# chrischoy/DeepGlobalRegistration

Hardware: AMD Instinct MI355X
Metric: pair registrations/sec (FCGF x2 + 1-NN + 6-D inlier net + gate + weighted Procrustes + SE(3) refinement) (higher is better)
Workload: dtype f32 results via 2 x f16 split operands (3 f16 MFMA products per MAC, f32 accumulate); k = 1 convs, kNN re-evaluation and registration in exact f32, SVD in f64

## Files before the change

### deepglobalregistration_amd/csrc/coordmap.hip

```cpp
#include <algorithm>

#include "dgr_internal.h"
#include "hash.h"

constexpr int SCAN_THREADS = 256;
constexpr int SCAN_ITEMS = 8;
constexpr int SCAN_BLOCK = SCAN_THREADS * SCAN_ITEMS;

__device__ __forceinline__ int block_exclusive_scan_256(int v, int *lds , int *total) {
  const int lane = threadIdx.x & 63, wave = threadIdx.x >> 6;
  int x = v;
#pragma unroll
  for (int d = 1; d < 64; d <<= 1) {
    int y = __shfl_up(x, d, 64);
    if (lane >= d) x += y;
  }
  if (lane == 63) lds[wave] = x;
  __syncthreads();
  int base = 0, tot = 0;
#pragma unroll
  for (int w = 0; w < SCAN_THREADS / 64; ++w) {
    int s = lds[w];
    if (w < wave) base += s;
    tot += s;
// ... 239 lines not shown
                            mask_out, stream);
  if (nc == 7)
    return unique_rows_t<7>(arena, keys, nullptr, n, first_flag, rank, n_unique_dev, table_out,
                            mask_out, stream);
  dgr_set_error("unsupported coordinate width %d", nc);
  return DGR_EINVAL;
}

template <int NC>
static int build_coord_maps_t(DgrArena &arena, const int32_t *coords, int64_t N, DgrMapSet *ms,
                              hipStream_t stream) {
  DgrCoordMap &c1 = ms->cm[0];
  c1.coords = const_cast<int32_t *>(coords);
  c1.n_cap = N;
  c1.ts = 1;
  DGR_ALLOC(c1.n_dev, arena, int32_t, 1);
  int32_t n32 = (int32_t)N;
  DGR_HIP_CHECK(hipMemcpyAsync(c1.n_dev, &n32, sizeof(int32_t), hipMemcpyHostToDevice, stream));
  {
    uint32_t cap = dgr_next_pow2((uint64_t)(2 * N > 64 ? 2 * N : 64));
    DGR_ALLOC(c1.table, arena, int32_t, cap);
    c1.table_mask = cap - 1;
    DGR_HIP_CHECK(hipMemsetAsync(c1.table, 0xff, (size_t)cap * sizeof(int32_t), stream));
    unique_insert<NC><<<grid_for(N), 256, 0, stream>>>(coords, nullptr, N, c1.table, cap - 1);
    unique_flag<NC><<<grid_for(N), 256, 0, stream>>>(coords, nullptr, N, c1.table, cap - 1, nullptr,
                                                    ms->overflow);
    DGR_LAUNCH_CHECK();
  }
  for (int l = 1; l < 4; ++l) {
    DgrCoordMap &p = ms->cm[l - 1];
    DgrCoordMap &c = ms->cm[l];
    c.ts = p.ts * 2;
    c.n_cap = p.n_cap;
    int32_t *keys, *flag, *rank;
    DGR_ALLOC(keys, arena, int32_t, p.n_cap * NC);
    DGR_ALLOC(flag, arena, int32_t, p.n_cap);
    DGR_ALLOC(rank, arena, int32_t, p.n_cap);
    DGR_ALLOC(c.coords, arena, int32_t, c.n_cap * NC);
    DGR_ALLOC(c.n_dev, arena, int32_t, 1);
    stride_keys<NC><<<grid_for(p.n_cap), 256, 0, stream>>>(p.coords, p.n_dev, c.ts, keys);
    DGR_CHECK(unique_rows_t<NC>(arena, keys, p.n_dev, p.n_cap, flag, rank, c.n_dev, &c.table,
                                &c.table_mask, stream));
    unique_compact<NC><<<grid_for(p.n_cap), 256, 0, stream>>>(keys, p.n_dev, p.n_cap, flag, rank,
                                                             c.coords, nullptr);
    table_relabel<<<grid_for((int64_t)c.table_mask + 1), 256, 0, stream>>>(c.table, c.table_mask + 1,
                                                                           rank);
    DGR_LAUNCH_CHECK();
  }
  return DGR_OK;
}

__global__ void half_keys_kernel(const int32_t *__restrict__ coords7, const int32_t *n_dev,
                                 int32_t *__restrict__ keys4) {
  int64_t r = (int64_t)blockIdx.x * blockDim.x + threadIdx.x;
  if (r >= *n_dev) return;
#pragma unroll
  for (int d = 0; d < 4; ++d) keys4[r * 4 + d] = coords7[r * 7 + d];
}

__global__ void bucket_count_kernel(const int32_t *__restrict__ keys4, const int32_t *n_dev,
                                    const int32_t *__restrict__ table, uint32_t mask,
                                    const int32_t *__restrict__ bkeys, int32_t *__restrict__ row_bucket,
                                    int32_t *counts) {
  int64_t r = (int64_t)blockIdx.x * blockDim.x + threadIdx.x;
  if (r >= *n_dev) return;
  int32_t q[4] = {keys4[r * 4], keys4[r * 4 + 1], keys4[r * 4 + 2], keys4[r * 4 + 3]};
  const int b = dgr_lookup<4>(table, mask, bkeys, q);
  row_bucket[r] = b;
  atomicAdd(&counts[b], 1);
}

__global__ void bucket_members_kernel(const int32_t *__restrict__ row_bucket, const int32_t *n_dev,
                                      const int32_t *__restrict__ start, int32_t *cursor, int32_t *__restrict__ members) {
  int64_t r = (int64_t)blockIdx.x * blockDim.x + threadIdx.x;
  if (r >= *n_dev) return;
  const int b = row_bucket[r];
  members[start[b] + atomicAdd(&cursor[b], 1)] = (int32_t)r;
}

__global__ void bucket_fill_kernel(const int32_t *__restrict__ row_bucket, const int32_t *n_dev,
                                   const int32_t *__restrict__ start, int32_t *cursor,
                                   const int32_t *__restrict__ members,
                                   const int32_t *__restrict__ coords7, int4 *__restrict__ second,
                                   int32_t *__restrict__ coords_new, int32_t *__restrict__ canon, int32_t *__restrict__ inv) {
  int64_t r = (int64_t)blockIdx.x * blockDim.x + threadIdx.x;
  if (r >= *n_dev) return;
  const int b = row_bucket[r];
  const int32_t *c = coords7 + r * 7;
  int p;
  if (members) {
    int rank = 0;
    for (int e = start[b], end = start[b + 1]; e < end; ++e) rank += members[e] < (int32_t)r;
    p = start[b] + rank;
  } else {
    p = start[b] + atomicAdd(&cursor[b], 1);
  }
  if (coords_new) {
#pragma unroll
    for (int d = 0; d < 7; ++d) coords_new[(int64_t)p * 7 + d] = c[d];
    canon[p] = (int32_t)r;
    inv[r] = p;
    second[p] = make_int4(c[4], c[5], c[6], p);
  } else {
    second[p] = make_int4(c[4], c[5], c[6], (int32_t)r);
  }
}

struct RenumberJobs {
  const int32_t *inv[4];
  int32_t *table[4];
  uint32_t cap[4];
};
__global__ void renumber_table_kernel(RenumberJobs j) {
  const int l = blockIdx.y;
  const uint32_t s = blockIdx.x * blockDim.x + threadIdx.x;
  if (s >= j.cap[l]) return;
  const int v = j.table[l][s];
  if (v >= 0) j.table[l][s] = j.inv[l][v];
}

int dgr_build_half_buckets(DgrArena &arena, DgrCoordMap *cm, DgrHalfBuckets *hb, int levels, int renumber_from,
                           hipStream_t stream) {
  DGR_REQUIRE(levels >= 1 && levels <= 4 && renumber_from >= 1, "half buckets: %d levels", levels);
  int32_t *keys[4], *flag[4], *rank[4], *nb_dev[4], *row_bucket[4], *counts[4], *cursor[4];
  uint32_t cap[4];
  size_t table_words = 0, count_words = 0;
  for (int l = 0; l < levels; ++l) {
    const int64_t n = cm[l].n_cap;
    cap[l] = dgr_next_pow2((uint64_t)(2 * n > 64 ? 2 * n : 64));
    table_words += cap[l];
    count_words += 2 * (size_t)(n + 1);
  }
  int32_t *tables, *cnts;
  DGR_ALLOC(tables, arena, int32_t, table_words);
  DGR_ALLOC(cnts, arena, int32_t, count_words);
  DGR_HIP_CHECK(hipMemsetAsync(tables, 0xff, table_words * sizeof(int32_t), stream));
  DGR_HIP_CHECK(hipMemsetAsync(cnts, 0, count_words * sizeof(int32_t), stream));
  for (int l = 0; l < levels; ++l) {
    const int64_t n = cm[l].n_cap;
    hb[l].table = tables; tables += cap[l];
    hb[l].mask = cap[l] - 1;
    counts[l] = cnts; cursor[l] = cnts + (n + 1); cnts += 2 * (n + 1);
    DGR_ALLOC(keys[l], arena, int32_t, n * 4);
    DGR_ALLOC(flag[l], arena, int32_t, n);
    DGR_ALLOC(rank[l], arena, int32_t, n);
    DGR_ALLOC(nb_dev[l], arena, int32_t, 1);
    DGR_ALLOC(row_bucket[l], arena, int32_t, n);
    DGR_ALLOC(hb[l].bkeys, arena, int32_t, n * 4);
    DGR_ALLOC(hb[l].start, arena, int32_t, n + 1);
    DGR_ALLOC(hb[l].second, arena, int4, n);
  }
  for (int l = 0; l < levels; ++l) {
    const int64_t n = cm[l].n_cap;
    half_keys_kernel<<<grid_for(n), 256, 0, stream>>>(cm[l].coords, cm[l].n_dev, keys[l]);
    unique_insert<4><<<grid_for(n), 256, 0, stream>>>(keys[l], cm[l].n_dev, n, hb[l].table, hb[l].mask);
    unique_flag<4><<<grid_for(n), 256, 0, stream>>>(keys[l], cm[l].n_dev, n, hb[l].table, hb[l].mask, flag[l], nullptr);
  }
  DGR_LAUNCH_CHECK();
  {
    const int32_t *ins[4];
    int32_t *outs[4], *tots[4];
    int64_t ns[4];
    for (int l = 0; l < levels; ++l) { ins[l] = flag[l]; outs[l] = rank[l]; tots[l] = nb_dev[l]; ns[l] = cm[l].n_cap; }
    DGR_CHECK(dgr_exclusive_scan_multi(arena, levels, ins, outs, ns, tots, stream));
  }
  for (int l = 0; l < levels; ++l) {
    const int64_t n = cm[l].n_cap;
    unique_compact<4><<<grid_for(n), 256, 0, stream>>>(keys[l], cm[l].n_dev, n, flag[l], rank[l], hb[l].bkeys, nullptr);
    table_relabel<<<grid_for((int64_t)hb[l].mask + 1), 256, 0, stream>>>(hb[l].table, hb[l].mask + 1, rank[l]);
    bucket_count_kernel<<<grid_for(n), 256, 0, stream>>>(keys[l], cm[l].n_dev, hb[l].table, hb[l].mask, hb[l].bkeys, row_bucket[l],
                                                         counts[l]);
  }
  DGR_LAUNCH_CHECK();
  {
    const int32_t *ins[4];
    int32_t *outs[4], *tots[4];
    int64_t ns[4];
    for (int l = 0; l < levels; ++l) { ins[l] = counts[l]; outs[l] = hb[l].start; tots[l] = nullptr; ns[l] = cm[l].n_cap + 1; }
    DGR_CHECK(dgr_exclusive_scan_multi(arena, levels, ins, outs, ns, tots, stream));
  }
  RenumberJobs rj = {};
  int nrj = 0;
  int64_t max_cap = 0;
  for (int l = 0; l < levels; ++l) {
    const int64_t n = cm[l].n_cap;
    int32_t *coords_new = nullptr, *canon = nullptr, *inv = nullptr;
    if (l >= renumber_from) {
      DGR_ALLOC(coords_new, arena, int32_t, n * 7);
      DGR_ALLOC(canon, arena, int32_t, n);
      DGR_ALLOC(inv, arena, int32_t, n);
      rj.inv[nrj] = inv; rj.table[nrj] = cm[l].table; rj.cap[nrj] = cm[l].table_mask + 1;
      max_cap = std::max<int64_t>(max_cap, rj.cap[nrj]);
      ++nrj;
    }
    const int32_t *members = nullptr;
    if (coords_new) {
      bucket_members_kernel<<<grid_for(n), 256, 0, stream>>>(row_bucket[l], cm[l].n_dev, hb[l].start, cursor[l], rank[l]);
      members = rank[l];
    }
    bucket_fill_kernel<<<grid_for(n), 256, 0, stream>>>(row_bucket[l], cm[l].n_dev, hb[l].start, cursor[l], members,
                                                        cm[l].coords, hb[l].second, coords_new, canon, inv);
    if (coords_new) { cm[l].coords = coords_new; cm[l].canon = canon; }
    hb[l].built = true;
  }
  if (nrj) renumber_table_kernel<<<dim3((unsigned)grid_for(max_cap), nrj), 256, 0, stream>>>(rj);
  DGR_LAUNCH_CHECK();
  return DGR_OK;
}

int dgr_build_coord_maps(DgrArena &arena, const int32_t *coords, int64_t N, DgrMapSet *ms,
                         hipStream_t stream) {
  if (ms->nc == 4) return build_coord_maps_t<4>(arena, coords, N, ms, stream);
  if (ms->nc == 7) return build_coord_maps_t<7>(arena, coords, N, ms, stream);
  dgr_set_error("unsupported dimension D=%d (3 and 6 are on the DGR path)", ms->D);
  return DGR_EINVAL;
}

template <typename T>
__global__ void voxel_keys(const T *__restrict__ xyz, int64_t M, T inv_unused, T voxel, int32_t batch,
                           int32_t *__restrict__ keys) {
  int64_t r = (int64_t)blockIdx.x * blockDim.x + threadIdx.x;
  if (r >= M) return;
  keys[r * 4] = batch;
#pragma unroll
  for (int d = 0; d < 3; ++d) keys[r * 4 + 1 + d] = (int32_t)floor(xyz[r * 3 + d] / voxel);
}

template <typename T>
__global__ void voxel_gather_xyz(const T *__restrict__ xyz, const int64_t *__restrict__ sel,
                                 const int32_t *n_dev, float *__restrict__ out) {
  int64_t r = (int64_t)blockIdx.x * blockDim.x + threadIdx.x;
  if (r >= *n_dev) return;
  int64_t s = sel[r];
#pragma unroll
  for (int d = 0; d < 3; ++d) out[r * 3 + d] = (float)xyz[s * 3 + d];
}

extern "C" int dgr_voxelize(dgr_ctx *ctx, const void *xyz, int is_f64, int64_t M, double voxel_size,
                            int32_t batch_index, int64_t *sel_out, int32_t *coords_out,
                            float *xyz_out, int64_t *n_out, dgr_stream stream_) {
  DGR_REQUIRE(ctx && xyz && sel_out && coords_out && n_out, "dgr_voxelize: NULL argument");
  DGR_REQUIRE(M > 0 && M < (1ll << 30), "dgr_voxelize: M=%lld out of range", (long long)M);
  DGR_REQUIRE(voxel_size > 0, "dgr_voxelize: voxel_size must be positive");
  hipStream_t stream = (hipStream_t)stream_;
  DGR_HIP_CHECK(hipSetDevice(ctx->device));
  DGR_CHECK(ctx->arena.reset());
  DgrArena &A = ctx->arena;
  int32_t *keys, *flag, *rank, *n_dev, *table;
  uint32_t mask;
  DGR_ALLOC(keys, A, int32_t, M * 4);
  DGR_ALLOC(flag, A, int32_t, M);
  DGR_ALLOC(rank, A, int32_t, M);
  DGR_ALLOC(n_dev, A, int32_t, 1);
  if (is_f64)
    voxel_keys<double><<<grid_for(M), 256, 0, stream>>>((const double *)xyz, M, 0.0, voxel_size,
                                                       batch_index, keys);
  else
    voxel_keys<float><<<grid_for(M), 256, 0, stream>>>((const float *)xyz, M, 0.f, (float)voxel_size,
                                                      batch_index, keys);
  DGR_CHECK(unique_rows_t<4>(A, keys, nullptr, M, flag, rank, n_dev, &table, &mask, stream));
  unique_compact<4><<<grid_for(M), 256, 0, stream>>>(keys, nullptr, M, flag, rank, coords_out, sel_out);
  if (xyz_out) {
    if (is_f64)
      voxel_gather_xyz<double><<<grid_for(M), 256, 0, stream>>>((const double *)xyz, sel_out, n_dev,
                                                               xyz_out);
    else
      voxel_gather_xyz<float><<<grid_for(M), 256, 0, stream>>>((const float *)xyz, sel_out, n_dev,
                                                              xyz_out);
  }
  DGR_LAUNCH_CHECK();
  int32_t n32 = 0;
  DGR_HIP_CHECK(hipMemcpyAsync(&n32, n_dev, sizeof(int32_t), hipMemcpyDeviceToHost, stream));
  DGR_HIP_CHECK(hipStreamSynchronize(stream));
  *n_out = n32;
  return DGR_OK;
}
```

### deepglobalregistration_amd/csrc/dgr_internal.h

```cpp
#pragma once
#include <hip/hip_runtime.h>
#include <stdint.h>
#include <stdio.h>
#include <stdlib.h>
#include <string>
#include <vector>

#include "../../include/dgr_hip.h"

void dgr_set_error(const char *fmt, ...);

#define DGR_HIP_CHECK(expr)                                                                  \
  do {                                                                                       \
    hipError_t _e = (expr);                                                                  \
    if (_e != hipSuccess) {                                                                  \
      dgr_set_error("%s:%d: %s failed: %s", __FILE__, __LINE__, #expr, hipGetErrorString(_e)); \
      return DGR_EHIP;                                                                       \
    }                                                                                        \
  } while (0)

#define DGR_CHECK(expr)          \
  do {                           \
    int _r = (expr);             \
    if (_r != DGR_OK) return _r; \
  } while (0)

#define DGR_REQUIRE(cond, ...)     \
  do {                             \
    if (!(cond)) {                 \
      dgr_set_error(__VA_ARGS__);  \
      return DGR_EINVAL;           \
    }                              \
  } while (0)

#define DGR_LAUNCH_CHECK() DGR_HIP_CHECK(hipGetLastError())

inline bool dgr_exact_f32() {
  static const bool on = getenv("DGR_EXACT_F32") != nullptr;
  return on;
}

struct DgrArena {
  struct Chunk {
    char *base;
    size_t size;
  };
  std::vector<Chunk> chunks;
  size_t cur = 0;
  size_t offset = 0;
  size_t high_water = 0, used_total = 0;
  uint64_t generation = 0;

  struct Mark {
    size_t cur, offset, used_total;
  };
  Mark mark() const { return {cur, offset, used_total}; }
  void rewind(const Mark &m) { cur = m.cur; offset = m.offset; used_total = m.used_total; }
  void *alloc(size_t bytes);
  int reset();
  void release();
  size_t reserved() const;
  template <typename T>
  T *get(size_t n) {
    return static_cast<T *>(alloc(n * sizeof(T)));
  }
};

#define DGR_ALLOC(ptr, arena, T, n)                       \
  do {                                                    \
    (ptr) = (arena).get<T>((size_t)(n) > 0 ? (size_t)(n) : 1); \
    if (!(ptr)) return DGR_ENOMEM;                        \
  } while (0)

constexpr int DGR_TILE_M = 64;

struct DgrCoordMap {
  int32_t *coords = nullptr;
  int32_t *n_dev = nullptr;
  int64_t n_cap = 0;
  int ts = 1;
  int32_t *table = nullptr;
  uint32_t table_mask = 0;
  int32_t *canon = nullptr;
};

struct DgrHalfBuckets {
  int32_t *bkeys = nullptr;
  int32_t *table = nullptr;
  uint32_t mask = 0;
  int32_t *start = nullptr;
  int4 *second = nullptr;
  bool built = false;
};

struct DgrKernelMap {
  int K = 0;
  int32_t *rule_ptr = nullptr;
  int32_t *tile_ptr = nullptr;
  int4 *tile_desc = nullptr;
  int64_t tile_cap = 0;
  int32_t *pair_in = nullptr;
  int32_t *pair_out = nullptr;
  int32_t *out_ptr = nullptr, *out_pos = nullptr;
  uint16_t *pair_k = nullptr;
  int32_t *in_ptr = nullptr, *in_pos = nullptr;
  int64_t pair_cap = 0;
  bool built = false;
};

constexpr int DGR_OS_ROWS = 64;
struct DgrNbrTable {
  int32_t *nbr = nullptr;
  int64_t n_pad = 0;
  int K = 27;
  bool built = false;
  int32_t *perm = nullptr, *cls_count = nullptr;
  int64_t cls_cap = 0;
};

struct DgrMapSet {
  int D = 3, nc = 4, conv1_ks = 3;
  bool use_nbr = false;
  DgrNbrTable nsame[4];
  DgrNbrTable ndown[3];
  DgrNbrTable nup[3];
  DgrCoordMap cm[4];
  DgrHalfBuckets hb[4];
  DgrKernelMap same[4];
  DgrKernelMap conv1;
  DgrKernelMap down[3];
  int32_t *overflow = nullptr;
};

int dgr_build_maps(DgrArena &arena, const int32_t *coords, int64_t N, int D, int conv1_ks,
                   DgrMapSet *ms, hipStream_t stream, bool skip_conv1_map = false, bool lean = false,
                   bool nbr_tables = false);
int dgr_nbr_counts(const DgrNbrTable &t, const int32_t *n_out_dev, int64_t counts[27]);
int dgr_conv1_probe(DgrArena &arena, const DgrCoordMap &cm, int ks, const float *in, int in_ld, int cin,
                    const float *w_tiled, const float *shift, float *out, int out_ld, int32_t *pair_count,
                    hipStream_t stream, const float *w_compact = nullptr, const char **kernel_name = nullptr,
                    uint32_t *out_amax = nullptr);
int dgr_unique_rows(DgrArena &arena, const int32_t *keys, int64_t n, int nc, int32_t *first_flag,
                    int32_t *rank, int32_t *n_unique_dev, int32_t **table_out, uint32_t *mask_out,
                    hipStream_t stream);
int dgr_exclusive_scan_i32(DgrArena &arena, const int32_t *in, int32_t *out, int64_t n,
                           int32_t *total_out, hipStream_t stream);
constexpr int DGR_SCAN_MAX = 24;
int dgr_exclusive_scan_multi(DgrArena &arena, int count, const int32_t *const *in, int32_t *const *out, const int64_t *n,
                             int32_t *const *total_out, hipStream_t stream);

struct DgrConvLaunch {
  const float *in;
  int in_ld;
  int in_relu;
  float *out;
  int out_ld;
  float *y;
  const float *shift;
  const float *w;
  int cin, cin_pad, cout, cout_pad, K;
  const int32_t *pair_in, *pair_out, *tile_ptr, *rule_ptr;
  const int4 *tile_desc;
  const int32_t *n_rows_dev;
  int64_t tile_bound;
  int l2_normalize = 0;
  unsigned long long *clk = nullptr;
};
int dgr_conv_launch(const DgrConvLaunch &a, int num_cus, hipStream_t stream, const char **kernel_name = nullptr);
struct DgrSplitRows {
  unsigned char *planes = nullptr;
  float *scale = nullptr;
  int channels = 0;
};
bool dgr_conv_wide_supported(int cin_pad, int cin, int cout);
// ... 136 lines not shown
```

### deepglobalregistration_amd/csrc/kmap.hip

```cpp
#include <string.h>

#include <algorithm>

#include "dgr_internal.h"
#include "hash.h"

constexpr int KM_THREADS = 256;

template <int D>
__device__ __forceinline__ void offset_of(int k, int ks, int ts, int32_t *delta) {
  const int half = ks >> 1;
#pragma unroll
  for (int d = 0; d < D; ++d) {
    delta[d] = ((k % ks) - half) * ts;
    k /= ks;
  }
}

template <int D>
__device__ __forceinline__ int probe(const int32_t *__restrict__ out_coords, int64_t o,
                                     const int32_t *delta, const int32_t *__restrict__ in_coords,
                                     const int32_t *__restrict__ in_table, uint32_t in_mask) {
  constexpr int NC = D + 1;
  int32_t q[NC];
// ... 19 lines not shown
  int32_t delta[D];
  offset_of<D>(k, ks, ts_in, delta);
  const int64_t o = (int64_t)rb * KM_THREADS + threadIdx.x;
  int hit = -1;
  if (o < n_out) {
    hit = probe<D>(out_coords, o, delta, in_coords, in_table, in_mask);
    hits[(int64_t)k * n_cap + o] = hit;
    if (hit >= 0) {
      atomicOr(&mask_out[o * KW + (k >> 5)], 1u << (k & 31));
      if (mask_in) atomicOr(&mask_in[(int64_t)hit * KW + (k >> 5)], 1u << (k & 31));
    }
  }
  unsigned long long m = __ballot(hit >= 0);
  if ((threadIdx.x & 63) == 0) wave_cnt[threadIdx.x >> 6] = __popcll(m);
  __syncthreads();
  if (threadIdx.x == 0) {
    int s = 0;
#pragma unroll
    for (int w = 0; w < KM_THREADS / 64; ++w) s += wave_cnt[w];
    block_counts[(int64_t)k * RB + rb] = s;
  }
}

__device__ __forceinline__ int mask_rank(const uint32_t *__restrict__ m, int k) {
  int r = 0;
  const int w = k >> 5;
  for (int i = 0; i < w; ++i) r += __popc(m[i]);
  return r + __popc(m[w] & ((1u << (k & 31)) - 1u));
}

__global__ void mask_count_kernel(const uint32_t *__restrict__ mask, int KW, const int32_t *n_dev, int64_t n_cap,
                                  int32_t *__restrict__ cnt, unsigned short *__restrict__ wpre = nullptr) {
  const int64_t r = (int64_t)blockIdx.x * blockDim.x + threadIdx.x;
  if (r >= n_cap) return;
  int c = 0;
  if (r < *n_dev)
    for (int i = 0; i < KW; ++i) {
      if (wpre) wpre[r * KW + i] = (unsigned short)c;
      c += __popc(mask[r * KW + i]);
    }
  cnt[r] = c;
}
constexpr int KM_MC_JOBS = 8;
struct MaskCountJobs {
  const uint32_t *mask[KM_MC_JOBS];
  const int32_t *n_dev[KM_MC_JOBS];
  long long n_cap[KM_MC_JOBS];
  int32_t *cnt[KM_MC_JOBS];
  unsigned short *wpre[KM_MC_JOBS];
};
template <int KW>
__global__ void mask_count_multi(MaskCountJobs J) {
  const int m = blockIdx.y;
  const int64_t r = (int64_t)blockIdx.x * blockDim.x + threadIdx.x;
  if (r >= J.n_cap[m]) return;
  int c = 0;
  if (r < *J.n_dev[m]) {
    uint32_t w[KW];
#pragma unroll
    for (int i = 0; i < KW; ++i) w[i] = J.mask[m][r * KW + i];
#pragma unroll
    for (int i = 0; i < KW; ++i) {
      J.wpre[m][r * KW + i] = (unsigned short)c;
      c += __popc(w[i]);
    }
  }
  J.cnt[m][r] = c;
}
__device__ __forceinline__ int mask_rank_pre(const uint32_t *__restrict__ m, const unsigned short *__restrict__ pre, int k) {
  return pre[k >> 5] + __popc(m[k >> 5] & ((1u << (k & 31)) - 1u));
}


__device__ __forceinline__ unsigned long long hit_pack(int k, int64_t o, int64_t in) {
  return ((unsigned long long)k << 54) | ((unsigned long long)o << 27) | (unsigned long long)in;
}
constexpr int KM_REGION = 512;
constexpr int KM_JOBS6 = 8;
struct HitList {
  unsigned long long *recs;
  int32_t *wave_count;
  int region;
};
__device__ __forceinline__ void hit_begin(volatile int *cur) {
  if ((threadIdx.x & 63) == 0) cur[threadIdx.x >> 6] = 0;
}
__device__ __forceinline__ int64_t hit_slots(int n, const HitList &h, volatile int *cur, int wave_id) {
  const unsigned long long act = __ballot(1), two = __ballot(n == 2);
  const int lane = threadIdx.x & 63, w = threadIdx.x >> 6;
  const unsigned long long below = (1ull << lane) - 1ull;
  int base = 0;
  if (lane == __ffsll((long long)act) - 1) {
    base = cur[w];
    const int need = __popcll(act) + __popcll(two);
    if (base >= 0 && base + need <= h.region) {
      cur[w] = base + need;
    } else {
      cur[w] = -1;
      base = -1;
    }
  }
  base = __builtin_amdgcn_readfirstlane(base);
  if (base < 0) return -1;
  return (int64_t)wave_id * h.region + base + __popcll(act & below) + __popcll(two & below);
}
__device__ __forceinline__ void hit_end(const HitList &h, volatile int *cur, int wave_id) {
  if ((threadIdx.x & 63) == 0) h.wave_count[wave_id] = cur[threadIdx.x >> 6];
}

struct PrunedArgs {
  const int32_t *out_coords, *n_out_dev;
  const int4 *out_order;
  int64_t n_cap;
  DgrHalfBuckets hb;
  int ts_in, symmetric;
};
template <class Emit>
__device__ __forceinline__ void pruned_search6(const PrunedArgs &a, int64_t t, Emit &&emit) {
  const int NJ = a.symmetric ? 14 : 27;
  const int ts_in = a.ts_in;
  const int ja = (int)(t / a.n_cap);
  const int64_t p = t - (int64_t)ja * a.n_cap;
  int b = -1;
  int64_t o = 0;
  int c4 = 0, c5 = 0, c6 = 0;
  if (ja < NJ && p < *a.n_out_dev) {
    const int4 me = a.out_order[p];
    o = me.w; c4 = me.x; c5 = me.y; c6 = me.z;
    const int32_t *co = a.out_coords + o * 7;
    int32_t q[4];
    q[0] = co[0];
    q[1] = co[1] + ((ja % 3) - 1) * ts_in;
    q[2] = co[2] + (((ja / 3) % 3) - 1) * ts_in;
    q[3] = co[3] + ((ja / 9) - 1) * ts_in;
    b = dgr_lookup<4>(a.hb.table, a.hb.mask, a.hb.bkeys, q);
  }
  const int beg = b >= 0 ? a.hb.start[b] : 0, end = b >= 0 ? a.hb.start[b + 1] : 0;
  for (int p0 = beg; p0 < end; p0 += 4) {
    int4 e[4];
#pragma unroll
    for (int u = 0; u < 4; ++u) e[u] = a.hb.second[min(p0 + u, end - 1)];
#pragma unroll
    for (int u = 0; u < 4; ++u) {
      if (p0 + u >= end) break;
      const int d4 = e[u].x - c4, d5 = e[u].y - c5, d6 = e[u].z - c6;
      if (abs(d4) <= ts_in && abs(d5) <= ts_in && abs(d6) <= ts_in) {
        const int k = ja + 27 * ((d4 / ts_in + 1) + 3 * (d5 / ts_in + 1) + 9 * (d6 / ts_in + 1));
        if (a.symmetric && ja == 13 && k > 364) continue;
        emit(k, o, e[u].w);
      }
    }
  }
}

struct Bits6Jobs {
  PrunedArgs pa[KM_JOBS6];
  uint32_t *mask_out[KM_JOBS6], *mask_in[KM_JOBS6];
  HitList hl[KM_JOBS6];
  int blocks[KM_JOBS6];
};
__global__ void __launch_bounds__(KM_THREADS)
    kmap_bits_pruned6(Bits6Jobs J, int KW) {
  __shared__ int hit_cur[KM_THREADS / 64];
  const int jm = blockIdx.y;
  if ((int)blockIdx.x >= J.blocks[jm]) return;
  const PrunedArgs a = J.pa[jm];
  uint32_t *const mask_out = J.mask_out[jm], *const mask_in = J.mask_in[jm];
  const HitList hl = J.hl[jm];
  hit_begin(hit_cur);
  const int wid = (int)(blockIdx.x * (KM_THREADS / 64) + (threadIdx.x >> 6));
  pruned_search6(a, (int64_t)blockIdx.x * KM_THREADS + threadIdx.x, [&](int k, int64_t o, int in) {
    atomicOr(&mask_out[o * KW + (k >> 5)], 1u << (k & 31));
    const int km = 728 - k;
    if (a.symmetric) {
      if (km != k) atomicOr(&mask_out[(int64_t)in * KW + (km >> 5)], 1u << (km & 31));
    } else if (mask_in) {
      atomicOr(&mask_in[(int64_t)in * KW + (k >> 5)], 1u << (k & 31));
    }
    const int n = (a.symmetric && km != k) ? 2 : 1;
    const int64_t s = hit_slots(n, hl, hit_cur, wid);
    if (s >= 0) {
      hl.recs[s] = hit_pack(k, o, in);
      if (n == 2) hl.recs[s + 1] = hit_pack(km, in, o);
    }
  });
  hit_end(hl, hit_cur, wid);
}

constexpr int KM_KMAX = 736;
struct Colmask6Jobs {
  const uint32_t *mask_out[KM_JOBS6];
  const int32_t *n_out_dev[KM_JOBS6];
  int RB[KM_JOBS6];
  int4 *cell[KM_JOBS6];
  int32_t *counts[KM_JOBS6], *row_cnt[KM_JOBS6];
  unsigned short *wpre[KM_JOBS6];
};
__global__ void __launch_bounds__(KM_THREADS)
    kmap_colmask(Colmask6Jobs J, int K, int KW) {
  __shared__ unsigned long long bal[KM_THREADS / 64][KM_KMAX];
  const int jm = blockIdx.y;
  const int RB = J.RB[jm];
  if ((int)blockIdx.x >= RB) return;
  const uint32_t *__restrict__ mask_out = J.mask_out[jm];
  const int32_t *n_out_dev = J.n_out_dev[jm];
  int4 *__restrict__ cell = J.cell[jm];
  int32_t *__restrict__ counts = J.counts[jm], *__restrict__ row_cnt = J.row_cnt[jm];
  unsigned short *__restrict__ wpre = J.wpre[jm];
  const int rb = blockIdx.x;
  const int lane = threadIdx.x & 63, wave = threadIdx.x >> 6;
  const int n_out = *n_out_dev;
  const int64_t o = (int64_t)rb * KM_THREADS + threadIdx.x;
  int row_pairs = 0;
  constexpr int KW_MAX = (KM_KMAX + 31) / 32;
  uint32_t words[KW_MAX];
#pragma unroll
  for (int w = 0; w < KW_MAX; ++w) words[w] = (w < KW && o < n_out) ? mask_out[o * KW + w] : 0u;
#pragma unroll
// ... 205 lines not shown
  if (need_in_csr) {
    DGR_ALLOC(km->in_ptr, arena, int32_t, n_in_cap + 1);
    DGR_ALLOC(km->in_pos, arena, int32_t, km->pair_cap);
  }
  return DGR_OK;
}

static void finalize_job(FinalizeJobs &fj, int m, const int32_t *base, const int32_t *total, int K, int RB, DgrKernelMap *km) {
  fj.base[m] = base; fj.total[m] = total; fj.K[m] = K; fj.RB[m] = RB;
  fj.rule_ptr[m] = km->rule_ptr; fj.tile_ptr[m] = km->tile_ptr;
  fj.desc[m] = km->tile_desc; fj.tile_cap[m] = km->tile_cap;
}

static int build_kernel_map3(DgrArena &arena, const DgrCoordMap &in, const DgrCoordMap &out, int ks, int max_pairs_per_row,
                             bool need_in_csr, bool want_pair_out, bool want_pair_k, DgrKernelMap *km,
                             int32_t *overflow, hipStream_t stream) {
  constexpr int D = 3;
  const int K = ks * ks * ks;
  const int64_t n_cap = out.n_cap, n_in_cap = in.n_cap;
  const int RB = (int)dgr_ceil_div(n_cap, KM_THREADS);
  DGR_CHECK(alloc_kernel_map(arena, K, n_cap, n_in_cap, max_pairs_per_row, need_in_csr, want_pair_out, want_pair_k, km));
  const int KW = (K + 31) / 32;
  DgrArena::Mark mk = arena.mark();
  int32_t *counts, *base, *total;
  DGR_ALLOC(counts, arena, int32_t, (int64_t)K * RB);
  DGR_ALLOC(base, arena, int32_t, (int64_t)K * RB);
  DGR_ALLOC(total, arena, int32_t, 1);
  uint32_t *mask_out, *mask_in = nullptr;
  int32_t *cnt_out, *cnt_in = nullptr;
  {
    const size_t w_out = (size_t)(n_cap + 1) * KW, w_in = need_in_csr ? (size_t)(n_in_cap + 1) * KW : 0;
    DGR_ALLOC(mask_out, arena, uint32_t, w_out + w_in);
    if (need_in_csr) mask_in = mask_out + w_out;
    DGR_HIP_CHECK(hipMemsetAsync(mask_out, 0, (w_out + w_in) * sizeof(uint32_t), stream));
  }
  DGR_ALLOC(cnt_out, arena, int32_t, n_cap + 1);
  if (need_in_csr) DGR_ALLOC(cnt_in, arena, int32_t, n_in_cap + 1);
  int32_t *hits;
  DGR_ALLOC(hits, arena, int32_t, (int64_t)K * n_cap);
  kmap_search<D><<<dim3(RB, K), KM_THREADS, 0, stream>>>(out.coords, out.n_dev, in.coords, in.table, in.table_mask, ks,
                                                         in.ts, RB, n_cap, hits, counts, KW, mask_out, mask_in);
  DGR_LAUNCH_CHECK();
  mask_count_kernel<<<(int)dgr_ceil_div(n_cap + 1, 256), 256, 0, stream>>>(mask_out, KW, out.n_dev, n_cap + 1, cnt_out);
  if (need_in_csr)
    mask_count_kernel<<<(int)dgr_ceil_div(n_in_cap + 1, 256), 256, 0, stream>>>(mask_in, KW, in.n_dev, n_in_cap + 1, cnt_in);
  {
    const int32_t *ins[3] = {cnt_out, counts, cnt_in};
    int32_t *outs[3] = {km->out_ptr, base, km->in_ptr}, *tots[3] = {nullptr, total, nullptr};
    const int64_t ns[3] = {n_cap + 1, (int64_t)K * RB, n_in_cap + 1};
    DGR_CHECK(dgr_exclusive_scan_multi(arena, need_in_csr ? 3 : 2, ins, outs, ns, tots, stream));
  }
  FinalizeJobs fj = {};
  finalize_job(fj, 0, base, total, K, RB, km);
  kmap_finalize<<<1, 1024, 0, stream>>>(fj);
  tile_desc_kernel<<<dim3((unsigned)dgr_ceil_div(km->tile_cap, 256), 1), 256, 0, stream>>>(fj);
  kmap_fill<<<dim3(RB, (K + KM_KGROUP - 1) / KM_KGROUP), KM_THREADS, 0, stream>>>(
      out.n_dev, RB, K, n_cap, hits, counts, base, km->pair_in, km->pair_out, km->pair_cap, overflow, KW, mask_out,
      km->out_ptr, km->out_pos, mask_in, km->in_ptr, km->in_pos, km->pair_k);
  DGR_LAUNCH_CHECK();
  arena.rewind(mk);
  km->built = true;
  return DGR_OK;
}

struct Kmap6Job {
  const DgrCoordMap *in, *out;
  const DgrHalfBuckets *hb;
  const DgrHalfBuckets *hb_out;
  bool need_in_csr, want_pair_out, want_pair_k;
  DgrKernelMap *km;
};
static int build_kernel_maps6(DgrArena &arena, const Kmap6Job *jobs, int nj, int max_pairs_per_row, int32_t *overflow,
                              hipStream_t stream) {
  constexpr int K = 729, KW = (K + 31) / 32;
  DGR_REQUIRE(nj >= 1 && nj <= KM_MAXJOBS, "6-D kernel maps: %d jobs", nj);
  struct Tr {
    int RB, symmetric;
    int64_t n_cap, n_in_cap, hit_waves;
    int32_t *counts, *base, *total, *cnt_out, *cnt_in;
    uint32_t *mask_out, *mask_in;
    int4 *cell;
    HitList hl;
    unsigned short *wpre_out, *wpre_in;
  } t[KM_MAXJOBS];
  for (int m = 0; m < nj; ++m) {
    const Kmap6Job &J = jobs[m];
    t[m].n_cap = J.out->n_cap; t[m].n_in_cap = J.in->n_cap;
    DGR_REQUIRE(t[m].n_cap < (1ll << 27) && t[m].n_in_cap < (1ll << 27), "6-D kernel maps: more than 2^27 rows");
    DGR_CHECK(alloc_kernel_map(arena, K, t[m].n_cap, t[m].n_in_cap, max_pairs_per_row, J.need_in_csr, J.want_pair_out,
                               J.want_pair_k, J.km));
  }
  DgrArena::Mark mk = arena.mark();
  {
    size_t words = 0;
    for (int m = 0; m < nj; ++m)
      words += (size_t)(t[m].n_cap + 1) * KW + (jobs[m].need_in_csr ? (size_t)(t[m].n_in_cap + 1) * KW : 0) + (size_t)(t[m].n_cap + 1);
    uint32_t *pool;
    DGR_ALLOC(pool, arena, uint32_t, words);
    DGR_HIP_CHECK(hipMemsetAsync(pool, 0, words * sizeof(uint32_t), stream));
    for (int m = 0; m < nj; ++m) {
      t[m].mask_out = pool; pool += (size_t)(t[m].n_cap + 1) * KW;
      t[m].mask_in = nullptr;
      if (jobs[m].need_in_csr) { t[m].mask_in = pool; pool += (size_t)(t[m].n_in_cap + 1) * KW; }
      t[m].cnt_out = reinterpret_cast<int32_t *>(pool); pool += (size_t)(t[m].n_cap + 1);
    }
  }
  for (int m = 0; m < nj; ++m) {
    const Kmap6Job &J = jobs[m];
    Tr &r = t[m];
    r.RB = (int)dgr_ceil_div(r.n_cap, KM_THREADS);
    r.symmetric = (J.in->coords == J.out->coords && !J.need_in_csr) ? 1 : 0;
    DGR_REQUIRE(J.hb && J.hb->built && J.hb_out && J.hb_out->built, "6-D kernel map: first-half buckets missing");
    DGR_ALLOC(r.counts, arena, int32_t, (int64_t)K * r.RB);
    DGR_ALLOC(r.base, arena, int32_t, (int64_t)K * r.RB);
    DGR_ALLOC(r.total, arena, int32_t, 1);
    r.cnt_in = nullptr;
    if (J.need_in_csr) DGR_ALLOC(r.cnt_in, arena, int32_t, r.n_in_cap + 1);
    DGR_ALLOC(r.cell, arena, int4, (int64_t)r.RB * (KM_THREADS / 64) * K);
    const int64_t search_blocks = dgr_ceil_div(r.n_cap * (r.symmetric ? 14 : 27), KM_THREADS);
    r.hit_waves = search_blocks * (KM_THREADS / 64);
    r.hl.region = (J.in->ts >= 8 && r.symmetric) ? 2 * KM_REGION : KM_REGION / 2;
    DGR_REQUIRE(r.hit_waves < (1ll << 31), "6-D kernel map: too many search waves");
    DGR_ALLOC(r.hl.recs, arena, unsigned long long, r.hit_waves * r.hl.region);
    DGR_ALLOC(r.hl.wave_count, arena, int32_t, r.hit_waves);
    DGR_ALLOC(r.wpre_out, arena, unsigned short, (r.n_cap + 1) * KW);
    r.wpre_in = nullptr;
    if (J.need_in_csr) DGR_ALLOC(r.wpre_in, arena, unsigned short, (r.n_in_cap + 1) * KW);
  }
  static_assert(KM_JOBS6 >= KM_MAXJOBS, "multi-job launch tables");
  {
    Bits6Jobs bj = {};
    Colmask6Jobs cj = {};
    int max_sb = 0, max_rb = 0;
    for (int m = 0; m < nj; ++m) {
      const Kmap6Job &J = jobs[m];
      Tr &r = t[m];
      bj.pa[m] = PrunedArgs{J.out->coords, J.out->n_dev, J.hb_out->second, r.n_cap, *J.hb, J.in->ts, r.symmetric};
      bj.mask_out[m] = r.mask_out; bj.mask_in[m] = r.mask_in; bj.hl[m] = r.hl;
      bj.blocks[m] = (int)(r.hit_waves / (KM_THREADS / 64));
      max_sb = std::max(max_sb, bj.blocks[m]);
      cj.mask_out[m] = r.mask_out; cj.n_out_dev[m] = J.out->n_dev; cj.RB[m] = r.RB; cj.cell[m] = r.cell;
      cj.counts[m] = r.counts; cj.row_cnt[m] = r.cnt_out; cj.wpre[m] = r.wpre_out;
      max_rb = std::max(max_rb, r.RB);
    }
    kmap_bits_pruned6<<<dim3((unsigned)max_sb, (unsigned)nj), KM_THREADS, 0, stream>>>(bj, KW);
    kmap_colmask<<<dim3((unsigned)max_rb, (unsigned)nj), KM_THREADS, 0, stream>>>(cj, K, KW);
    {
      MaskCountJobs mj = {};
      int nm = 0;
      long long max_rows = 0;
      for (int m = 0; m < nj; ++m)
        if (jobs[m].need_in_csr) {
          mj.mask[nm] = t[m].mask_in; mj.n_dev[nm] = jobs[m].in->n_dev; mj.n_cap[nm] = t[m].n_in_cap + 1;
          mj.cnt[nm] = t[m].cnt_in; mj.wpre[nm] = t[m].wpre_in;
          max_rows = std::max(max_rows, mj.n_cap[nm]);
          ++nm;
        }
      static_assert(KM_MC_JOBS >= KM_MAXJOBS, "mask-count job table");
      if (nm) mask_count_multi<KW><<<dim3((unsigned)dgr_ceil_div(max_rows, 256), (unsigned)nm), 256, 0, stream>>>(mj);
    }
  }
  DGR_LAUNCH_CHECK();
  {
    const int32_t *ins[DGR_SCAN_MAX];
    int32_t *outs[DGR_SCAN_MAX], *tots[DGR_SCAN_MAX];
    int64_t ns[DGR_SCAN_MAX];
    int c = 0;
    for (int m = 0; m < nj; ++m) {
      ins[c] = t[m].cnt_out; outs[c] = jobs[m].km->out_ptr; tots[c] = nullptr; ns[c++] = t[m].n_cap + 1;
      ins[c] = t[m].counts; outs[c] = t[m].base; tots[c] = t[m].total; ns[c++] = (int64_t)K * t[m].RB;
      if (jobs[m].need_in_csr) { ins[c] = t[m].cnt_in; outs[c] = jobs[m].km->in_ptr; tots[c] = nullptr; ns[c++] = t[m].n_in_cap + 1; }
    }
    DGR_CHECK(dgr_exclusive_scan_multi(arena, c, ins, outs, ns, tots, stream));
  }
  FinalizeJobs fj = {};
  int64_t max_tiles = 0;
  for (int m = 0; m < nj; ++m) {
    finalize_job(fj, m, t[m].base, t[m].total, K, t[m].RB, jobs[m].km);
    max_tiles = std::max<int64_t>(max_tiles, jobs[m].km->tile_cap);
  }
  kmap_finalize<<<nj, 1024, 0, stream>>>(fj);
  tile_desc_kernel<<<dim3((unsigned)dgr_ceil_div(max_tiles, 256), nj), 256, 0, stream>>>(fj);
  {
    Place6Jobs pj = {};
    int max_pb = 0;
    for (int m = 0; m < nj; ++m) {
      const Kmap6Job &J = jobs[m];
      Tr &r = t[m];
      DgrKernelMap *km = J.km;
      pj.p[m] = PlaceArgs{K, KW, r.RB, r.mask_out, km->out_ptr, r.cell, r.base, km->pair_in, km->pair_out, km->pair_k, km->out_pos,
                          km->pair_cap, overflow, r.mask_in, km->in_ptr, km->in_pos, r.wpre_out, r.wpre_in};
      pj.replay[m] = PrunedArgs{J.out->coords, J.out->n_dev, J.hb_out->second, r.n_cap, *J.hb, J.in->ts, r.symmetric};
      pj.h[m] = r.hl;
      pj.n_waves[m] = (int)r.hit_waves;
      pj.blocks[m] = (int)std::min<int64_t>(dgr_ceil_div(r.hit_waves, KM_THREADS / 64), 16384);
      max_pb = std::max(max_pb, pj.blocks[m]);
      km->built = true;
    }
    kmap_place_hits<<<dim3((unsigned)max_pb, (unsigned)nj), KM_THREADS, 0, stream>>>(pj);
  }
  DGR_LAUNCH_CHECK();
  arena.rewind(mk);
  return DGR_OK;
}

constexpr int NBR_JOBS = 10;
struct NbrJobs {
  const int32_t *out_coords[NBR_JOBS], *n_out_dev[NBR_JOBS], *in_coords[NBR_JOBS], *in_table[NBR_JOBS];
  uint32_t in_mask[NBR_JOBS];
  int ts[NBR_JOBS];
  long long n_pad[NBR_JOBS];
  int32_t *nbr[NBR_JOBS];
};
__global__ void __launch_bounds__(KM_THREADS) nbr_search3(NbrJobs J) {
  const int jm = blockIdx.z;
  const int64_t n_pad = J.n_pad[jm];
  const int64_t o = (int64_t)blockIdx.x * KM_THREADS + threadIdx.x;
  if (o >= n_pad) return;
  int32_t *__restrict__ nbr = J.nbr[jm];
  const int kz = blockIdx.y;
  if (o >= *J.n_out_dev[jm]) {
#pragma unroll
    for (int u = 0; u < 9; ++u) nbr[(int64_t)(9 * kz + u) * n_pad + o] = -1;
    return;
  }
  const int sts = J.ts[jm];
  const int4 c = *reinterpret_cast<const int4 *>(J.out_coords[jm] + o * 4);
  int32_t q[9][4];
#pragma unroll
  for (int u = 0; u < 9; ++u) {
    q[u][0] = c.x;
    q[u][1] = c.y + ((u % 3) - 1) * sts;
    q[u][2] = c.z + ((u / 3) - 1) * sts;
    q[u][3] = c.w + (kz - 1) * sts;
  }
  int hit[9];
  dgr_lookup_many<4, 9>(J.in_table[jm], J.in_mask[jm], J.in_coords[jm], q, hit);
#pragma unroll
  for (int u = 0; u < 9; ++u) nbr[(int64_t)(9 * kz + u) * n_pad + o] = hit[u];
}

struct ClsJobs {
  const int32_t *coords[3], *n_dev[3];
  int ts[3], nb[3];
  int32_t *blk_cnt[3], *perm[3], *cls_count[3];
  long long cls_cap[3];
};
__device__ __forceinline__ int parity_class(const int32_t *coords, int64_t o, int ts) {
  const int4 c = *reinterpret_cast<const int4 *>(coords + o * 4);
  return ((c.y / ts) & 1) | (((c.z / ts) & 1) << 1) | (((c.w / ts) & 1) << 2);
}
__global__ void __launch_bounds__(KM_THREADS) cls_count_kernel(ClsJobs J) {
  __shared__ int wcnt[KM_THREADS / 64][8];
  const int l = blockIdx.y, b = blockIdx.x;
  if (b >= J.nb[l]) return;
  const int64_t o = (int64_t)b * KM_THREADS + threadIdx.x;
  const int cls = o < *J.n_dev[l] ? parity_class(J.coords[l], o, J.ts[l]) : 8;
#pragma unroll
  for (int c = 0; c < 8; ++c) {
    const unsigned long long m = __ballot(cls == c);
    if ((threadIdx.x & 63) == 0) wcnt[threadIdx.x >> 6][c] = __popcll(m);
  }
  __syncthreads();
  if (threadIdx.x < 8) {
    int n = 0;
    for (int w = 0; w < KM_THREADS / 64; ++w) n += wcnt[w][threadIdx.x];
    J.blk_cnt[l][b * 8 + threadIdx.x] = n;
  }
}
__global__ void __launch_bounds__(KM_THREADS) cls_fill_kernel(ClsJobs J) {
  __shared__ int part[KM_THREADS / 64][8], before[8], wcnt[KM_THREADS / 64][8];
  const int l = blockIdx.y, b = blockIdx.x;
  if (b >= J.nb[l]) return;
  const int lane = threadIdx.x & 63, wave = threadIdx.x >> 6;
  int acc[8] = {0, 0, 0, 0, 0, 0, 0, 0};
// ... 319 lines not shown
```

Baseline: 392.2.

## Precompute per-bucket neighbor lookups for 6-D kernel map search

Adds a kernel that, for each unique half-key bucket and each neighbor offset, looks up the neighbor bucket in the input hash table once and stores it in a table. The pruned 6-D search and its replay in the placement pass then read this table through a new position-to-bucket array, instead of re-hashing per output point. This removes duplicated hash probes shared by points in the same bucket and avoids the probes being done twice, at the cost of an extra launch and extra memory. It also replaces the volatile LDS slot counter in the hit list with workgroup-scope atomic fetch-add, and records overflow when the list ends.

```diff
diff --git a/deepglobalregistration_amd/csrc/coordmap.hip b/deepglobalregistration_amd/csrc/coordmap.hip
--- a/deepglobalregistration_amd/csrc/coordmap.hip
+++ b/deepglobalregistration_amd/csrc/coordmap.hip
@@ -345,6 +345,7 @@
                                    const int32_t *__restrict__ start, int32_t *cursor,
                                    const int32_t *__restrict__ members,
                                    const int32_t *__restrict__ coords7, int4 *__restrict__ second,
+                                   int32_t *__restrict__ pos_bucket,
                                    int32_t *__restrict__ coords_new, int32_t *__restrict__ canon, int32_t *__restrict__ inv) {
   int64_t r = (int64_t)blockIdx.x * blockDim.x + threadIdx.x;
   if (r >= *n_dev) return;
@@ -358,6 +359,7 @@
   } else {
     p = start[b] + atomicAdd(&cursor[b], 1);
   }
+  pos_bucket[p] = b;
   if (coords_new) {
 #pragma unroll
     for (int d = 0; d < 7; ++d) coords_new[(int64_t)p * 7 + d] = c[d];
@@ -412,6 +414,8 @@
     DGR_ALLOC(hb[l].bkeys, arena, int32_t, n * 4);
     DGR_ALLOC(hb[l].start, arena, int32_t, n + 1);
     DGR_ALLOC(hb[l].second, arena, int4, n);
+    DGR_ALLOC(hb[l].pos_bucket, arena, int32_t, n);
+    hb[l].n_buckets_dev = nb_dev[l];
   }
   for (int l = 0; l < levels; ++l) {
     const int64_t n = cm[l].n_cap;
@@ -462,7 +466,7 @@
       members = rank[l];
     }
     bucket_fill_kernel<<<grid_for(n), 256, 0, stream>>>(row_bucket[l], cm[l].n_dev, hb[l].start, cursor[l], members,
-                                                        cm[l].coords, hb[l].second, coords_new, canon, inv);
+                                                        cm[l].coords, hb[l].second, hb[l].pos_bucket, coords_new, canon, inv);
     if (coords_new) { cm[l].coords = coords_new; cm[l].canon = canon; }
     hb[l].built = true;
   }
diff --git a/deepglobalregistration_amd/csrc/dgr_internal.h b/deepglobalregistration_amd/csrc/dgr_internal.h
--- a/deepglobalregistration_amd/csrc/dgr_internal.h
+++ b/deepglobalregistration_amd/csrc/dgr_internal.h
@@ -90,6 +90,8 @@
   uint32_t mask = 0;
   int32_t *start = nullptr;
   int4 *second = nullptr;
+  int32_t *pos_bucket = nullptr;
+  int32_t *n_buckets_dev = nullptr;
   bool built = false;
 };
 
diff --git a/deepglobalregistration_amd/csrc/kmap.hip b/deepglobalregistration_amd/csrc/kmap.hip
--- a/deepglobalregistration_amd/csrc/kmap.hip
+++ b/deepglobalregistration_amd/csrc/kmap.hip
@@ -125,39 +125,65 @@
   int32_t *wave_count;
   int region;
 };
-__device__ __forceinline__ void hit_begin(volatile int *cur) {
-  if ((threadIdx.x & 63) == 0) cur[threadIdx.x >> 6] = 0;
-}
-__device__ __forceinline__ int64_t hit_slots(int n, const HitList &h, volatile int *cur, int wave_id) {
+__device__ __forceinline__ void hit_begin(int *cur) {
+  if ((threadIdx.x & 63) == 0) __hip_atomic_store(&cur[threadIdx.x >> 6], 0, __ATOMIC_RELAXED, __HIP_MEMORY_SCOPE_WORKGROUP);
+}
+__device__ __forceinline__ int64_t hit_slots(int n, const HitList &h, int *cur, int wave_id) {
   const unsigned long long act = __ballot(1), two = __ballot(n == 2);
   const int lane = threadIdx.x & 63, w = threadIdx.x >> 6;
   const unsigned long long below = (1ull << lane) - 1ull;
   int base = 0;
   if (lane == __ffsll((long long)act) - 1) {
-    base = cur[w];
     const int need = __popcll(act) + __popcll(two);
-    if (base >= 0 && base + need <= h.region) {
-      cur[w] = base + need;
-    } else {
-      cur[w] = -1;
-      base = -1;
-    }
+    base = __hip_atomic_fetch_add(&cur[w], need, __ATOMIC_RELAXED, __HIP_MEMORY_SCOPE_WORKGROUP);
+    if (base + need > h.region) base = -1;
   }
   base = __builtin_amdgcn_readfirstlane(base);
   if (base < 0) return -1;
   return (int64_t)wave_id * h.region + base + __popcll(act & below) + __popcll(two & below);
 }
-__device__ __forceinline__ void hit_end(const HitList &h, volatile int *cur, int wave_id) {
-  if ((threadIdx.x & 63) == 0) h.wave_count[wave_id] = cur[threadIdx.x >> 6];
+__device__ __forceinline__ void hit_end(const HitList &h, int *cur, int wave_id) {
+  if ((threadIdx.x & 63) == 0) {
+    const int n = __hip_atomic_load(&cur[threadIdx.x >> 6], __ATOMIC_RELAXED, __HIP_MEMORY_SCOPE_WORKGROUP);
+    h.wave_count[wave_id] = n <= h.region ? n : -1;
+  }
 }
 
 struct PrunedArgs {
-  const int32_t *out_coords, *n_out_dev;
+  const int32_t *n_out_dev;
   const int4 *out_order;
+  const int32_t *out_bucket;
+  const int32_t *nb;
   int64_t n_cap;
   DgrHalfBuckets hb;
   int ts_in, symmetric;
 };
+
+struct NbTable6Jobs {
+  const int32_t *out_bkeys[KM_JOBS6], *n_buckets_dev[KM_JOBS6];
+  const int32_t *table[KM_JOBS6], *bkeys[KM_JOBS6];
+  uint32_t mask[KM_JOBS6];
+  int32_t *nb[KM_JOBS6];
+  long long n_cap[KM_JOBS6];
+  int ts_in[KM_JOBS6], NJ[KM_JOBS6];
+};
+__global__ void __launch_bounds__(KM_THREADS) kmap_nb_table6(NbTable6Jobs J) {
+  const int jm = blockIdx.y;
+  const int64_t n_cap = J.n_cap[jm];
+  const int64_t t = (int64_t)blockIdx.x * KM_THREADS + threadIdx.x;
+  const int ja = (int)(t / n_cap);
+  const int64_t B = t - (int64_t)ja * n_cap;
+  if (ja >= J.NJ[jm] || B >= *J.n_buckets_dev[jm]) return;
+  const int ts_in = J.ts_in[jm];
+  const int4 key = *reinterpret_cast<const int4 *>(J.out_bkeys[jm] + B * 4);
+  int32_t q[4];
+  q[0] = key.x;
+  q[1] = key.y + ((ja % 3) - 1) * ts_in;
+  q[2] = key.z + (((ja / 3) % 3) - 1) * ts_in;
+  q[3] = key.w + ((ja / 9) - 1) * ts_in;
+  J.nb[jm][t] = dgr_lookup<4>(J.table[jm], J.mask[jm], J.bkeys[jm], q);
+}
+
 template <class Emit>
 __device__ __forceinline__ void pruned_search6(const PrunedArgs &a, int64_t t, Emit &&emit) {
   const int NJ = a.symmetric ? 14 : 27;
@@ -169,14 +195,9 @@
   int c4 = 0, c5 = 0, c6 = 0;
   if (ja < NJ && p < *a.n_out_dev) {
     const int4 me = a.out_order[p];
+    const int B = a.out_bucket[p];
     o = me.w; c4 = me.x; c5 = me.y; c6 = me.z;
-    const int32_t *co = a.out_coords + o * 7;
-    int32_t q[4];
-    q[0] = co[0];
-    q[1] = co[1] + ((ja % 3) - 1) * ts_in;
-    q[2] = co[2] + (((ja / 3) % 3) - 1) * ts_in;
-    q[3] = co[3] + ((ja / 9) - 1) * ts_in;
-    b = dgr_lookup<4>(a.hb.table, a.hb.mask, a.hb.bkeys, q);
+    b = a.nb[(int64_t)ja * a.n_cap + B];
   }
   const int beg = b >= 0 ? a.hb.start[b] : 0, end = b >= 0 ? a.hb.start[b + 1] : 0;
   for (int p0 = beg; p0 < end; p0 += 4) {
@@ -548,6 +569,8 @@
     int4 *cell;
     HitList hl;
     unsigned short *wpre_out, *wpre_in;
+    int32_t *nb;
+    PrunedArgs pa;
   } t[KM_MAXJOBS];
   for (int m = 0; m < nj; ++m) {
     const Kmap6Job &J = jobs[m];
@@ -592,16 +615,22 @@
     DGR_ALLOC(r.wpre_out, arena, unsigned short, (r.n_cap + 1) * KW);
     r.wpre_in = nullptr;
     if (J.need_in_csr) DGR_ALLOC(r.wpre_in, arena, unsigned short, (r.n_in_cap + 1) * KW);
+    DGR_ALLOC(r.nb, arena, int32_t, r.n_cap * (r.symmetric ? 14 : 27));
+    r.pa = PrunedArgs{J.out->n_dev, J.hb_out->second, J.hb_out->pos_bucket, r.nb, r.n_cap, *J.hb, J.in->ts, r.symmetric};
   }
   static_assert(KM_JOBS6 >= KM_MAXJOBS, "multi-job launch tables");
   {
     Bits6Jobs bj = {};
     Colmask6Jobs cj = {};
+    NbTable6Jobs tj = {};
     int max_sb = 0, max_rb = 0;
     for (int m = 0; m < nj; ++m) {
       const Kmap6Job &J = jobs[m];
       Tr &r = t[m];
-      bj.pa[m] = PrunedArgs{J.out->coords, J.out->n_dev, J.hb_out->second, r.n_cap, *J.hb, J.in->ts, r.symmetric};
+      tj.out_bkeys[m] = J.hb_out->bkeys; tj.n_buckets_dev[m] = J.hb_out->n_buckets_dev;
+      tj.table[m] = J.hb->table; tj.bkeys[m] = J.hb->bkeys; tj.mask[m] = J.hb->mask;
+      tj.nb[m] = r.nb; tj.n_cap[m] = r.n_cap; tj.ts_in[m] = J.in->ts; tj.NJ[m] = r.symmetric ? 14 : 27;
+      bj.pa[m] = r.pa;
       bj.mask_out[m] = r.mask_out; bj.mask_in[m] = r.mask_in; bj.hl[m] = r.hl;
       bj.blocks[m] = (int)(r.hit_waves / (KM_THREADS / 64));
       max_sb = std::max(max_sb, bj.blocks[m]);
@@ -609,6 +638,7 @@
       cj.counts[m] = r.counts; cj.row_cnt[m] = r.cnt_out; cj.wpre[m] = r.wpre_out;
       max_rb = std::max(max_rb, r.RB);
     }
+    kmap_nb_table6<<<dim3((unsigned)max_sb, (unsigned)nj), KM_THREADS, 0, stream>>>(tj);
     kmap_bits_pruned6<<<dim3((unsigned)max_sb, (unsigned)nj), KM_THREADS, 0, stream>>>(bj, KW);
     kmap_colmask<<<dim3((unsigned)max_rb, (unsigned)nj), KM_THREADS, 0, stream>>>(cj, K, KW);
     {
@@ -656,7 +686,7 @@
       DgrKernelMap *km = J.km;
       pj.p[m] = PlaceArgs{K, KW, r.RB, r.mask_out, km->out_ptr, r.cell, r.base, km->pair_in, km->pair_out, km->pair_k, km->out_pos,
                           km->pair_cap, overflow, r.mask_in, km->in_ptr, km->in_pos, r.wpre_out, r.wpre_in};
-      pj.replay[m] = PrunedArgs{J.out->coords, J.out->n_dev, J.hb_out->second, r.n_cap, *J.hb, J.in->ts, r.symmetric};
+      pj.replay[m] = r.pa;
       pj.h[m] = r.hl;
       pj.n_waves[m] = (int)r.hit_waves;
       pj.blocks[m] = (int)std::min<int64_t>(dgr_ceil_div(r.hit_waves, KM_THREADS / 64), 16384);
```

Result: no change. 393.2 (median of 2 runs) (+0.3%).
